# debbiemarkslab/EVcouplings

Measured on AMD Instinct MI355X. Metric: plmc L-BFGS iterations/sec (PLM fit, synthetic MSA), higher is better.
Workload: dtype f32 (forward: f16 hi/lo split couplings on the 2:4 sparse MFMA, f32 accumulation -- in the last iterations of a fit 39-bit fixed-point couplings as five int8 digit planes, exact; backward: 24-bit fixed-point residuals as three int8 digit planes on the int8 MFMA (32-bit / four there), exact int32 acc; 1 GPU; headline: synthetic MSA L=300 q=21 N=50000, theta=0.8, lambda_h=0.01, lambda_J=59.8; parallelism=single GPU

## Files before the change

evcouplings_amd/csrc/plm_host.cpp:

```cpp
#include "../../include/plm_hip.h"
#include "plm_internal.h"
#include "plm_host_util.h"
#include "plm_lbfgs.h"

#include <algorithm>
#include <chrono>
#include <cmath>
#include <cstdarg>
#include <cstdio>
#include <cstdlib>
#include <cstring>
#include <string>
#include <vector>

namespace {

thread_local std::string g_err;

int fail(int code, const char *fmt, ...) {
    char buf[512];
    va_list ap;
    va_start(ap, fmt);
    vsnprintf(buf, sizeof buf, fmt, ap);
    va_end(ap);
// ... 307 lines not shown
    if (d.nblk_own > 0) PLM_HIP(plm_launch_backward(d, c->msa_cm, c->Rt, c->G, nullptr, c->st));
    PLM_HIP(plm_launch_pack_g(d, c->G, c->gsend, c->st));
    PLM_TRY(ctx_collective(c, PLM_COLL_ALLTOALL, c->gsend, c->ghalo, c->g_send.data(), c->g_recv.data()));
    PLM_TRY(group_norms(c));
    PLM_HIP(plm_launch_assemble(d, c->G, d.ksplit, c->ghalo, c->x, c->g, c->prob.lambda_h, c->prob.lambda_j,
                                c->reg_part, 0, 0.f, c->pair_n2, (float)c->prob.lambda_group, c->st));
    PLM_HIP(plm_launch_finish_fx(d, c->fx_part, c->n_fx_part(), nullptr, 0, c->reg_part, plm_reg_parts(d), c->scal,
                                 c->st));
    c->n_evals++;
    return PLM_OK;
}

int ctx_eval_enqueue(plm_ctx *c) {
    const PlmDims &d = c->d;
    if (d.sharded) return ctx_eval_enqueue_sharded(c);
    PLM_HIP(plm_launch_maxabs(d, c->x, c->maxbits, c->jexp, c->st));
    PLM_HIP(plm_launch_expand(d, c->x, nullptr, c->jexp, c->Bt, c->fwd_accurate ? 1 : 0, c->st));
    PLM_TRY(forward_at_x(c));
    PLM_HIP(plm_launch_backward(d, c->msa_cm, c->Rt, c->G, nullptr, c->st));
    const void *Gsrc = c->G;
    int ks_count = d.ksplit, n_shard_nll = 0;
    const double *shard_nll = nullptr;
    if (d.nshards > 1) {
        const size_t slab = plm_slab_bytes(d);
        char *mine = (char *)c->gather + (size_t)d.shard * slab;
        PLM_HIP(plm_launch_slab_reduce(d, c->G, (float *)mine, c->st));
        PLM_HIP(plm_launch_partial_sum(c->fx_part, c->n_fx_part(), (double *)(mine + slab - 256), c->st));
        PLM_HIP(hipStreamSynchronize(c->st));
        if (!c->exchange) return fail(PLM_EINVAL, "n_shards > 1 but no exchange callback set");
        if (c->exchange(c->gather, slab, d.nshards, d.shard, c->exchange_user) != 0)
            return fail(PLM_ECALLBACK, "exchange callback failed");
        Gsrc = c->gather;
        ks_count = 0;
        n_shard_nll = d.nshards;
        shard_nll = (const double *)((char *)c->gather + slab - 256);
    }
    PLM_TRY(group_norms(c));
    PLM_HIP(plm_launch_assemble(d, Gsrc, ks_count, nullptr, c->x, c->g, c->prob.lambda_h, c->prob.lambda_j,
                                c->reg_part, 0, 0.f, c->pair_n2, (float)c->prob.lambda_group, c->st));
    PLM_HIP(plm_launch_finish_fx(d, c->fx_part, c->n_fx_part(), shard_nll, n_shard_nll, c->reg_part,
                                 plm_reg_parts(d), c->scal, c->st));
    c->n_evals++;
    return PLM_OK;
}

bool vp_enabled(const plm_ctx *c) {
    return !(c->prob.flags & PLM_FLAG_JOINT_LBFGS) && (c->d.nshards == 1 || c->d.sharded) && c->prob.lambda_h > 0;
}
int vp_alloc(plm_ctx *c) {
    if (c->hj) return PLM_OK;
    const size_t nsites = (size_t)std::max(std::max(1, (c->d.b16_hi - c->d.b16_lo) * 16),
                                           std::min(c->d.L, c->d.own_hi * 16) - c->d.h_site0);
    PLM_TRY(plm_dalloc((char **)&c->hj, plm_hj_bytes(c->d)));
    PLM_TRY(plm_dalloc((char **)&c->hpart, plm_hpart_bytes(c->d)));
    PLM_TRY(plm_dalloc((char **)&c->gpart, plm_gpart_bytes(c->d)));
    PLM_TRY(plm_dalloc((char **)&c->dpart, plm_gpart_bytes(c->d)));
    PLM_TRY(plm_dalloc(&c->hg2, nsites));
    PLM_TRY(plm_dalloc(&c->hinv, nsites * c->d.Q * c->d.Q));
    PLM_TRY(plm_dalloc(&c->h64, 2 * plm_h64_stride(c->d)));
    PLM_TRY(plm_dalloc(&c->hcnt, plm_h64_stride(c->d)));
    c->hcnt_valid = false;
    PLM_TRY(plm_dalloc((char **)&c->vp_flag, sizeof(PlmVpState)));
    PLM_HIP(hipMemsetAsync(c->vp_flag, 0, sizeof(PlmVpState), c->st));
    for (auto &e : c->vp_ev) PLM_HIP(hipEventCreate(&e));
    for (auto &e : c->gemm_ev) PLM_HIP(hipEventCreate(&e));
    c->vp_hess_age = -1;
    return PLM_OK;
}
int vp_counts(plm_ctx *c) {
    if (!c->hcnt_valid) {
        PLM_HIP(plm_launch_site_counts(c->d, c->msa_cm, c->w, c->hcnt, c->st));
        c->hcnt_valid = true;
    }
    return PLM_OK;
}
int vp_stage1(plm_ctx *c) {
    const PlmDims &d = c->d;
    PLM_TRY(vp_counts(c));
    if (d.sharded) {
        PLM_TRY(ctx_collective(c, PLM_COLL_ALLTOALL, x_rectangles(c), c->xhalo, c->x_send.data(), c->x_recv.data()));
        PLM_HIP(plm_launch_maxabs2(c->x + d.nh_pad_l, d.n_local - d.nh_pad_l, c->xhalo,
                                   d.nx_halo * (int64_t)PLM_BLOCK_FLOATS(d), c->maxbits, c->jexp, d.jexp_bias, c->st));
        PLM_HIP(plm_launch_expand(d, c->x, c->xhalo, c->jexp, c->Bt, c->fwd_accurate ? 1 : 0, c->st));
    } else {
        PLM_HIP(plm_launch_maxabs(d, c->x, c->maxbits, c->jexp, c->st));
        PLM_HIP(plm_launch_expand(d, c->x, nullptr, c->jexp, c->Bt, c->fwd_accurate ? 1 : 0, c->st));
    }
    if (c->gemm_ev[0]) PLM_HIP(hipEventRecord(c->gemm_ev[0], c->st));
    PLM_HIP(plm_launch_forward_store(d, c->msa_rm, c->Bt, c->jexp, c->hj, c->fwd_accurate, c->st));
    PLM_HIP(plm_launch_h64_init(d, c->x, c->h64, c->st));
    return PLM_OK;
}
int vp_counts(plm_ctx *c);
int vp_step_and_residuals(plm_ctx *c, bool refresh) {
    const PlmDims &d = c->d;
    PLM_TRY(vp_counts(c));
    const int full = (refresh || c->vp_hess_age < 0) ? 1 : 0;
    PLM_HIP(plm_launch_hpass(d, c->hj, c->msa_rm, c->w, c->h64, 0, full ? 2 : 1, c->fwd_accurate, nullptr, nullptr, c->hpart,
                             c->gpart, c->dpart, nullptr, PLM_VP_ALWAYS, c->st));
    PLM_HIP(plm_launch_hsolve(d, c->hpart, c->gpart, full, c->x, c->h64, c->prob.lambda_h, 1, c->hinv, c->hg2, c->scal + 5, 0.0,
                              0.0, nullptr, 0, c->hcnt, c->dpart, c->st));
    if (full) c->vp_hess_age = 0;
    PLM_HIP(plm_launch_hpass(d, c->hj, c->msa_rm, c->w, c->h64, 1, 1, c->fwd_accurate, c->Rt, c->fx_part, c->hpart, c->gpart,
                             nullptr, nullptr, PLM_VP_ALWAYS, c->st));
    PLM_HIP(plm_launch_hsolve(d, c->hpart, c->gpart, 0, c->x, c->h64, c->prob.lambda_h, 0, c->hinv, c->hg2, c->scal + 5, 0.0,
                              0.0, nullptr, 0, c->hcnt, c->dpart, c->st));
    return PLM_OK;
// ... 992 lines not shown
        hipError_t e = hipEventRecord(ev[0], c->st);
        if (e == hipSuccess) e = plm_launch_hpass(d, c->hj, c->msa_rm, c->w, c->h64, 0, 2, 0, nullptr, nullptr, c->hpart, c->gpart, c->dpart,
                                                  nullptr, PLM_VP_ALWAYS, c->st);
        if (e == hipSuccess) e = plm_launch_hsolve(d, c->hpart, c->gpart, 1, c->x, c->h64, c->prob.lambda_h, 1, c->hinv, c->hg2, c->scal + 5,
                                                   0.0, 0.0, nullptr, 0, c->hcnt, c->dpart, c->st);
        if (e == hipSuccess) e = hipEventRecord(ev[1], c->st);
        if (e == hipSuccess) e = plm_launch_hpass(d, c->hj, c->msa_rm, c->w, c->h64, 1, 1, 0, c->Rt, c->fx_part, c->hpart, c->gpart, nullptr,
                                                  nullptr, PLM_VP_ALWAYS, c->st);
        if (e == hipSuccess) e = plm_launch_hsolve(d, c->hpart, c->gpart, 0, c->x, c->h64, c->prob.lambda_h, 0, c->hinv, c->hg2, c->scal + 5,
                                                   0.0, 0.0, nullptr, 0, c->hcnt, c->dpart, c->st);
        if (e == hipSuccess) e = hipEventRecord(ev[2], c->st);
        if (e == hipSuccess) e = hipEventSynchronize(ev[2]);
        if (e == hipSuccess && hipEventElapsedTime(&ms, ev[0], ev[1]) == hipSuccess) acc[0] += ms;
        if (e == hipSuccess && hipEventElapsedTime(&ms, ev[1], ev[2]) == hipSuccess) acc[1] += ms;
        if (e != hipSuccess) rc = fail(PLM_EDEVICE, "field position timing: %s", hipGetErrorString(e));
    }
    for (auto &e : ev) (void)hipEventDestroy(e);
    c->vp_hess_age = 0;
    out_ms[0] = (float)(acc[0] / reps);
    out_ms[1] = (float)(acc[1] / reps);
    return rc;
}

static int field_probe_checks(plm_ctx_t *c) {
    if (!c->have_weights) return fail(PLM_EINVAL, "weights not set");
    if (c->d.nshards != 1 || c->d.sharded) return fail(PLM_EUNSUPPORTED, "the field-solver probes run on single-shard contexts");
    if (!vp_enabled(c)) return fail(PLM_EINVAL, "the field-solver probes need a variable-projection context (not joint, lambda_h > 0)");
    return PLM_OK;
}
int plm_ctx_field_position(plm_ctx_t *c, int32_t role, int32_t accurate, int32_t update, int32_t prefill,
                           plm_field_buffers_t *out) {
    if (!c || !out) return fail(PLM_EINVAL, "NULL argument");
    if (role < PLM_FIELD_ROLE_STATS || role > PLM_FIELD_ROLE_RESIDUAL) return fail(PLM_EINVAL, "unknown role %d", (int)role);
    if (!out->gpart || !out->dpart || !out->hpart || !out->hcnt || !out->hinv || !out->g2_site || !out->g2_sum || !out->h64 ||
        !out->nll_part)
        return fail(PLM_EINVAL, "NULL output buffer");
    PLM_TRY(field_probe_checks(c));
    const PlmDims &d = c->d;
    const int64_t nsites = (int64_t)(d.b16_hi - d.b16_lo) * 16, hs = (int64_t)plm_h64_stride(d);
    const int64_t n_g = (int64_t)(plm_gpart_bytes(d) / sizeof(double)), n_h = (int64_t)(plm_hpart_bytes(d) / sizeof(float));
    if (out->n_gpart != n_g || out->n_hpart != n_h || out->n_hcnt != hs || out->n_hinv != nsites * d.Q * d.Q ||
        out->n_g2_site != nsites || out->n_h64 != 2 * hs || out->n_nll_part != c->n_fx_part())
        return fail(PLM_EINVAL, "output buffer sizes do not match the context");
    PLM_HIP(hipSetDevice(c->device));
    PLM_TRY(vp_alloc(c));
    const int full = role == PLM_FIELD_ROLE_HESSIAN ? 1 : 0;
    if (!full && update && c->vp_hess_age < 0) return fail(PLM_EINVAL, "no cached inverse Hessians: run a Hessian position first");
    c->eval_valid = false;
    ctx_set_accurate(c, accurate != 0);
    PLM_TRY(vp_stage1(c));
    if (prefill) {
        PLM_HIP(hipMemsetAsync(c->gpart, 0xFF, plm_gpart_bytes(d), c->st));
        PLM_HIP(hipMemsetAsync(c->dpart, 0xFF, plm_gpart_bytes(d), c->st));
        PLM_HIP(hipMemsetAsync(c->hpart, 0xFF, plm_hpart_bytes(d), c->st));
        PLM_HIP(hipMemsetAsync(c->fx_part, 0xFF, sizeof(double) * c->n_fx_part(), c->st));
        PLM_HIP(hipMemsetAsync(c->h64 + hs, 0xFF, sizeof(double) * hs, c->st));
    }
    if (role == PLM_FIELD_ROLE_RESIDUAL)
        PLM_HIP(plm_launch_hpass(d, c->hj, c->msa_rm, c->w, c->h64, 1, 1, c->fwd_accurate, c->Rt, c->fx_part, c->hpart, c->gpart,
                                 nullptr, nullptr, PLM_VP_ALWAYS, c->st));
    else
        PLM_HIP(plm_launch_hpass(d, c->hj, c->msa_rm, c->w, c->h64, 0, full ? 2 : 1, c->fwd_accurate, nullptr, nullptr, c->hpart,
                                 c->gpart, c->dpart, nullptr, PLM_VP_ALWAYS, c->st));
    PLM_HIP(plm_launch_hsolve(d, c->hpart, c->gpart, full, c->x, c->h64, c->prob.lambda_h, update ? 1 : 0, c->hinv, c->hg2,
                              c->scal + 5, 0.0, 0.0, nullptr, 0, c->hcnt, c->dpart, c->st));
    if (full) c->vp_hess_age = 0;
    PLM_HIP(hipMemcpyAsync(out->gpart, c->gpart, sizeof(double) * n_g, hipMemcpyDeviceToHost, c->st));
    PLM_HIP(hipMemcpyAsync(out->dpart, c->dpart, sizeof(double) * n_g, hipMemcpyDeviceToHost, c->st));
    PLM_HIP(hipMemcpyAsync(out->hpart, c->hpart, sizeof(float) * n_h, hipMemcpyDeviceToHost, c->st));
    PLM_HIP(hipMemcpyAsync(out->hcnt, c->hcnt, sizeof(double) * hs, hipMemcpyDeviceToHost, c->st));
    PLM_HIP(hipMemcpyAsync(out->hinv, c->hinv, sizeof(double) * nsites * d.Q * d.Q, hipMemcpyDeviceToHost, c->st));
    PLM_HIP(hipMemcpyAsync(out->g2_site, c->hg2, sizeof(double) * nsites, hipMemcpyDeviceToHost, c->st));
    PLM_HIP(hipMemcpyAsync(out->g2_sum, c->scal + 5, sizeof(double), hipMemcpyDeviceToHost, c->st));
    PLM_HIP(hipMemcpyAsync(out->h64, c->h64, sizeof(double) * 2 * hs, hipMemcpyDeviceToHost, c->st));
    PLM_HIP(hipMemcpyAsync(out->nll_part, c->fx_part, sizeof(double) * c->n_fx_part(), hipMemcpyDeviceToHost, c->st));
    PLM_HIP(hipStreamSynchronize(c->st));
    return PLM_OK;
}
int plm_ctx_field_solve(plm_ctx_t *c, double tol, int32_t vp_c_prev, int32_t invalidate, int32_t accurate,
                        plm_field_solve_t *res, double *fields, int64_t n_fields) {
    if (!c || !res || !fields) return fail(PLM_EINVAL, "NULL argument");
    if (!(tol >= 0) || vp_c_prev < 0 || vp_c_prev > 11) return fail(PLM_EINVAL, "tol must be >= 0 and vp_c_prev in 0..11");
    PLM_TRY(field_probe_checks(c));
    const PlmDims &d = c->d;
    const int64_t hs = (int64_t)plm_h64_stride(d);
    if (n_fields != hs) return fail(PLM_EINVAL, "fields must hold %lld doubles", (long long)hs);
    static_assert(PLM_FIELD_HIST == PLM_VP_HIST && PLM_FIELD_MAXBLK == PLM_VP_MAXBLK, "plm_field_solve_t mirrors PlmVpState");
    PLM_HIP(hipSetDevice(c->device));
    PLM_TRY(vp_alloc(c));
    c->eval_valid = false;
    ctx_set_accurate(c, accurate != 0);
    c->vp_floor2 = ctx_vp_floor2(c);
    c->vp_c_prev = vp_c_prev;
    if (invalidate) c->vp_hess_age = -1;
    const double tol2 = tol * tol;
    double gh2 = 0;
    PLM_TRY(ctx_eval_vp_run(c, tol2, [&]() -> int { return fetch_scalars(c, 0, 8); }, &gh2));
    PlmVpState S;
    PLM_HIP(hipMemcpyAsync(&S, c->vp_flag, sizeof S, hipMemcpyDeviceToHost, c->st));
    PLM_HIP(hipStreamSynchronize(c->st));
    PLM_HIP(hipMemcpyAsync(fields, c->h64 + (size_t)(S.cur ? hs : 0), sizeof(double) * hs, hipMemcpyDeviceToHost, c->st));
    PLM_HIP(hipStreamSynchronize(c->st));
    memset(res, 0, sizeof *res);
    res->gh2 = gh2;
    res->fx = c->h_scal[0];
    res->nll = c->h_scal[1];
    res->passes = (int32_t)std::lround(c->h_scal[6]);
// ... 659 lines not shown
```

evcouplings_amd/csrc/plm_internal.h:

```cpp
#pragma once
#include <stdint.h>
#include <stddef.h>
#include <hip/hip_runtime.h>

#define PLM_MAX_SHARDS 16
#define PLM_PAD_STATE 127
#define PLM_SEQ_TILE 256
#define PLM_R_EXP 14
#define PLM_BWD_MAXPLANES 4
#define PLM_R_QMAX3 8355000.0f
#define PLM_R_QMAX4 2138000000.0f
#define PLM_BWD_KSTEP 128
#define PLM_BWDW_COLS 9
#define PLM_BWD_ONEHOT_VALUE (-128)

#define PLM_FWD_NG(Q) (((Q) + 2) / 4)
#define PLM_FWD_SPU(Q) (4 * PLM_FWD_NG(Q))
#define PLM_FWD_TILES(Q) (5 * PLM_FWD_NG(Q))

struct PlmDims {
    int N, L, Q;
    int Qc;
    int Np;
    int nb16;
// ... 130 lines not shown
                               hipStream_t st);
hipError_t plm_launch_onehot_rt(const PlmDims &d, const int8_t *msa_rm, const float *w, void *Rt,
                                hipStream_t st);
hipError_t plm_launch_maxabs(const PlmDims &d, const float *x, uint32_t *maxbits, int32_t *jexp,
                             hipStream_t st);
hipError_t plm_launch_expand(const PlmDims &d, const float *x, const float *xhalo, const int32_t *jexp,
                             void *Bt, int exact, hipStream_t st);
hipError_t plm_launch_forward_energy(const PlmDims &d, const int8_t *msa_rm, const void *Bt, const float *x,
                                     const int32_t *jexp, int potentials, int accurate, float *out, hipStream_t st);
hipError_t plm_launch_energy_sum(const PlmDims &d, const float *part, double *out, hipStream_t st);
hipError_t plm_launch_forward_store(const PlmDims &d, const int8_t *msa_rm, const void *Bt, const int32_t *jexp,
                                    float *hj, int exact, hipStream_t st);
int plm_fwd_groups(int q, int exact);
hipError_t plm_launch_hpass(const PlmDims &d, const float *hj, const int8_t *msa_rm, const float *w,
                            const double *h64, int write_rt, int stats, int exact, void *Rt, double *fx_part, float *hpart,
                            double *gpart, double *dpart, const int *state, int cond, hipStream_t st);
#define PLM_VP_HIST 24
#define PLM_VP_MAXBLK 256
struct PlmVpState {
    int done;
    int want_rt;
    int final_skip;
    int passes;
    int cur;
    int pad_;
    double g2_prev;
    double g2_prev2;
    double hist[PLM_VP_HIST];
    int hist_loud[PLM_VP_HIST];
    unsigned char quiet[PLM_VP_MAXBLK];
};
#define PLM_VP_ALWAYS 0
#define PLM_VP_PASS 1
#define PLM_VP_PASS_RT 2
#define PLM_VP_FINAL 3
hipError_t plm_launch_vp_reset(int *state, int want_rt, double *zero3, hipStream_t st);
struct PlmRccl;
int plm_rccl_id(void *id128);
int plm_rccl_version();
int plm_rccl_init(const void *id128, int nranks, int rank, PlmRccl **out);
void plm_rccl_destroy(PlmRccl *p);
int plm_rccl_collective(PlmRccl *p, int op, void *send, void *recv, const int64_t *scounts, const int64_t *rcounts,
                        hipStream_t st);
const char *plm_rccl_error();
hipError_t plm_launch_h64_init(const PlmDims &d, const float *x, double *h64, hipStream_t st);
hipError_t plm_launch_hsolve(const PlmDims &d, const float *hpart, const double *gpart, int full, float *x, double *h64,
                             double lambda_h, int update, double *hinv, double *g2_site, double *g2_out, double tol2,
                             double floor2, int *state, int chain, const double *cnt, const double *dpart, hipStream_t st);
hipError_t plm_launch_site_counts(const PlmDims &d, const int8_t *msa_cm, const float *w, double *cnt, hipStream_t st);
size_t plm_h64_stride(const PlmDims &d);
hipError_t plm_launch_fields_to_x(const PlmDims &d, const double *h64, const int *state, float *x, hipStream_t st);
size_t plm_hj_bytes(const PlmDims &d);
size_t plm_hpart_bytes(const PlmDims &d);
size_t plm_gpart_bytes(const PlmDims &d);
hipError_t plm_launch_backward(const PlmDims &d, const int8_t *msa_cm, const void *Rt, int32_t *G, const int *run,
                               hipStream_t st);
hipError_t plm_launch_slab_reduce(const PlmDims &d, const int32_t *G, float *slab, hipStream_t st);
hipError_t plm_launch_assemble(const PlmDims &d, const void *G, int ks_count, const float *ghalo,
                               const float *x, float *g, float lambda_h, float lambda_j, double *reg_part,
                               int mode, float inv_neff, const float *pair_n2, float lambda_g, hipStream_t st);
hipError_t plm_launch_pair_norms(const PlmDims &d, const float *x, float *n2, hipStream_t st);
#define PLM_BLOCK_FLOATS(d) ((size_t)(d).Q * (d).Q * 256)
hipError_t plm_launch_pack_g(const PlmDims &d, const int32_t *G, float *sendbuf, hipStream_t st);
hipError_t plm_launch_maxabs2(const float *a, int64_t na, const float *b, int64_t nb, uint32_t *maxbits,
                              int32_t *jexp, int jexp_bias, hipStream_t st);
hipError_t plm_launch_finish_fx(const PlmDims &d, const double *fx_part, int n_fx_part,
                                const double *shard_nll, int n_shard_nll, const double *reg_part,
                                int n_reg_part, double *out2 , hipStream_t st);
hipError_t plm_launch_partial_sum(const double *part, int n, double *out, hipStream_t st);
#define PLM_DOT_BLOCKS 1024
hipError_t plm_launch_dots(int npairs, const float *const *a, const float *const *b, int64_t n,
                           double *scratch, double *out, hipStream_t st);
hipError_t plm_launch_lincomb(float *out, float ca, const float *a, float cb, const float *b,
                              int64_t n, hipStream_t st);
hipError_t plm_launch_canon_to_native(const PlmDims &d, const float *xc, float *xn, hipStream_t st);
hipError_t plm_launch_native_to_canon(const PlmDims &d, const float *xn, float *xc, hipStream_t st);
hipError_t plm_launch_fn(const PlmDims &d, const float *jij_canon, float *fn, int a_lo, int g_lo, hipStream_t st);
hipError_t plm_launch_msa_columns(const PlmDims &d, const int8_t *msa_rm, int8_t *msa_cm, int cm_rows, hipStream_t st);
hipError_t plm_launch_compact_gap_blocks(const PlmDims &d, const float *blocks, float *out, hipStream_t st);
hipError_t plm_launch_gap_normalise_pairs(const PlmDims &d, float *fij_canon, double fixed_total, hipStream_t st);
hipError_t plm_launch_align_stats(const int8_t *msa, int n, int L, int gap_state, const int8_t *query, int32_t *seq_gaps,
                                  int32_t *col_gaps, int32_t *ident, hipStream_t st);
size_t plm_bt_bytes(const PlmDims &d);
size_t plm_rt_bytes(const PlmDims &d);
size_t plm_g_bytes(const PlmDims &d);
size_t plm_slab_bytes(const PlmDims &d);
int plm_reg_parts(const PlmDims &d);
bool plm_q_supported(int q);
int plm_q_template(int q);
void plm_pick_tile(int q, int *fm, int *fn);

#define PLM_MAX_BASIS 42
struct PlmVecList {
    const float *v[PLM_MAX_BASIS];
    int n;
};
hipError_t plm_launch_multidot(const PlmVecList &queries, const PlmVecList &basis, int64_t n, double *scratch,
                               double *out, const float *dinv, unsigned wq, unsigned long long wb, hipStream_t st);
struct PlmCoefList {
    float c[PLM_MAX_BASIS];
};
hipError_t plm_launch_multiaxpy(float *out, const PlmVecList &basis, const PlmCoefList &coef, int64_t n,
                                const float *dinv, int first_weighted, hipStream_t st);
hipError_t plm_launch_precond(const PlmDims &d, const float *fv, float neff, float lambda_h, float lambda_j, float *dinv,
                              hipStream_t st);
hipError_t plm_launch_sy_multidot(float *s_new, float *y_new, const float *x, const float *xp, const float *g, const float *gp,
// ... 7 lines not shown
```

evcouplings_amd/csrc/plm_kernels.hip:

```cpp
#include "../../include/plm_hip.h"
#include "plm_internal.h"
#include <math.h>
#include <stdlib.h>
#include <string.h>
#include <mutex>
#include <utility>

typedef _Float16 half8 __attribute__((ext_vector_type(8)));
typedef _Float16 half4 __attribute__((ext_vector_type(4)));
typedef _Float16 half16 __attribute__((ext_vector_type(16)));
typedef float f32x4 __attribute__((ext_vector_type(4)));
typedef int i32x4 __attribute__((ext_vector_type(4)));
typedef unsigned int u32;

#ifndef PLM_DMA_STAGGER_FWD
#define PLM_DMA_STAGGER_FWD 4
#endif
#ifndef PLM_DMA_STAGGER_BWD
#define PLM_DMA_STAGGER_BWD 0
#endif
typedef unsigned long long u64;
#ifndef PLM_ASYNC_A
#define PLM_ASYNC_A 1
#endif
// ... 1123 lines not shown
#define PLM_HSTATS(Q) ((Q) + (Q) * ((Q) + 1) / 2)
__host__ __device__ constexpr int plm_qc_min(int Q) { return Q == 4 ? 2 : Q == 5 ? 5 : Q == 20 ? 6 : Q == 21 ? 21 : 22; }
#ifndef PLM_HESS_SAMPLE
#define PLM_HESS_SAMPLE 32
#endif
#ifndef PLM_NEWTON_CAP
#define PLM_NEWTON_CAP 3.0
#endif
__device__ __forceinline__ float sum_over_g(float v) {
    unsigned u = __float_as_uint(v);
    auto a = __builtin_amdgcn_permlane32_swap(u, u, false, false);
    v = __uint_as_float(a[0]) + __uint_as_float(a[1]);
    u = __float_as_uint(v);
    auto b = __builtin_amdgcn_permlane16_swap(u, u, false, false);
    return __uint_as_float(b[0]) + __uint_as_float(b[1]);
}
__device__ __forceinline__ float log_unbiased(float z) {
    const float l2 = __builtin_amdgcn_logf(z);
    return __builtin_fmaf(l2, -1.904654323148236e-9f, l2 * 0.693147182464599609375f);
}
__device__ __forceinline__ float sel_eq(int x, int a, float if_ne, float if_eq) {
    float out;
    asm("v_cmp_eq_u32 vcc, %1, %2\n\tv_cndmask_b32 %0, %3, %4, vcc" : "=v"(out) : "s"(a), "v"(x), "v"(if_ne), "v"(if_eq) : "vcc");
    return out;
}
__device__ __forceinline__ void sel_eq2(int x, int a, float ne0, float eq0, float ne1, float eq1, float &o0, float &o1) {
    asm("v_cmp_eq_u32 vcc, %2, %3\n\tv_cndmask_b32 %0, %4, %5, vcc\n\tv_cndmask_b32 %1, %6, %7, vcc"
        : "=&v"(o0), "=&v"(o1) : "s"(a), "v"(x), "v"(ne0), "v"(eq0), "v"(ne1), "v"(eq1) : "vcc");
}
__global__ void k_sum_partials(const double *__restrict__ p, int n, double *out);
struct HpassArgs {
    const float4 *hj;
    const int8_t *msa_rm;
    const float *w;
    const double *h;
    int hstride;
    char *Rt;
    double *fx_part;
    float *hpart;
    double *gpart;
    float rscale;
    double *dpart;
    const int *state;
    int cond;
    int sel;
};
__device__ __forceinline__ bool vp_runs(const int *state, int cond) {
    if (!state || cond == PLM_VP_ALWAYS) return true;
    const PlmVpState *S = (const PlmVpState *)state;
    if (cond == PLM_VP_FINAL) return S->final_skip == 0;
    if (S->done) return false;
    return cond == PLM_VP_PASS_RT ? S->want_rt != 0 : S->want_rt == 0;
}
#define PLM_HESS_PARTS(Q) (((Q) == 20 || (Q) == 21) ? 3 : 1)
template <int Q> __host__ __device__ constexpr int hess_entry0(int a) { return a * Q - a * (a - 1) / 2; }
template <int Q> __host__ __device__ constexpr int hess_row_begin(int part) {
    if (part <= 0) return 0;
    if (part >= PLM_HESS_PARTS(Q)) return Q;
    int a = 0;
    while (a < Q && hess_entry0<Q>(a) * PLM_HESS_PARTS(Q) < part * (Q * (Q + 1) / 2)) a++;
    return a;
}
template <int Q> __host__ __device__ constexpr int hess_part_entries() {
    int m = 0;
    for (int p = 0; p < PLM_HESS_PARTS(Q); p++) {
        const int n = hess_entry0<Q>(hess_row_begin<Q>(p + 1)) - hess_entry0<Q>(hess_row_begin<Q>(p));
        m = n > m ? n : m;
    }
    return m;
}
template <int Q, bool WRITE_RT, int STATS, bool XACT>
__global__ __launch_bounds__(512) void k_hpass(PlmDims d, HpassArgs A) {
    extern __shared__ __attribute__((aligned(16))) char smem[];
    constexpr int NH = (STATS == 2) ? Q * (Q + 1) / 2 : 0;
    constexpr int NSP = (STATS == 2) ? PLM_HESS_PARTS(Q) : 1;
    constexpr int NHP = (STATS == 2) ? hess_part_entries<Q>() : 0;
    if (!vp_runs(A.state, A.cond)) return;
    if (A.state) A.h += (size_t)((const PlmVpState *)A.state)->cur * A.hstride;
    const int tid = threadIdx.x, lane = tid & 63;
    const int wave = __builtin_amdgcn_readfirstlane(tid >> 6);
    const int ns1 = (d.nstiles + PLM_HESS_SAMPLE - 1) / PLM_HESS_SAMPLE;
    const int sel = A.sel;
    const int part = (int)blockIdx.x % NSP, bid = (int)blockIdx.x / NSP;
    int row_lo = 0, row_hi = Q;
    if constexpr (NSP > 1) {
        row_lo = part == 0 ? 0 : (part == 1 ? hess_row_begin<Q>(1) : hess_row_begin<Q>(2));
        row_hi = part == 0 ? hess_row_begin<Q>(1) : (part == 1 ? hess_row_begin<Q>(2) : Q);
    }
    const int ent_lo = row_lo * Q - row_lo * (row_lo - 1) / 2, ent_hi = row_hi * Q - row_hi * (row_hi - 1) / 2;
    const int nst = sel == 0 ? d.nstiles : (sel == 1 ? ns1 : d.nstiles - ns1);
    const int kt = bid % nst, b16l = bid / nst;
    if (A.state && A.cond == PLM_VP_PASS && b16l < PLM_VP_MAXBLK && ((const PlmVpState *)A.state)->quiet[b16l]) return;
    const int stile = sel == 0 ? kt : (sel == 1 ? kt * PLM_HESS_SAMPLE : kt + kt / (PLM_HESS_SAMPLE - 1) + 1);
    constexpr int HW = Q > 21 ? 2 : 8;
    constexpr bool sampled = STATS == 2, DIAG = STATS == 3 || (STATS == 2 && Q > 21);
    const int blk = b16l * d.nstiles + stile;
    const int b16 = d.b16_lo + b16l;
    const int r = lane & 15, g = lane >> 4;
    const int s_wave = stile * PLM_SEQ_TILE + wave * 32;
    const int gap = d.gap_mode;
    const int i = b16 * 16 + r;
    const bool site_ok = i < d.L;
    float hv[XACT ? 1 : Q], hl[XACT ? 1 : Q];
    double hd[XACT ? Q : 1];
    auto load_fields = [&](bool opaque) {
        u32 hoff = (u32)(site_ok ? i - d.h_site0 : 0) * Q;
        if (opaque) asm volatile("" : "+v"(hoff));
#pragma unroll
        for (int a = 0; a < Q; a++) {
            const double h64 = site_ok ? A.h[hoff + a] : 0.0;
            if constexpr (XACT) {
                hd[a] = h64;
            } else {
                hv[a] = (float)h64;
                hl[a] = (float)(h64 - (double)hv[a]);
            }
        }
    };
    constexpr bool LDSF = !WRITE_RT && !XACT && (STATS != 2 || Q > 21);
    constexpr size_t STAT_BYTES = (size_t)16 * (8 * Q * sizeof(double) * (DIAG ? 2 : 1) + HW * NHP * sizeof(float));
    float2 *lf = (float2 *)(smem + STAT_BYTES);
    constexpr bool FAST = !WRITE_RT && !XACT && (STATS == 1 || STATS == 3);
    if constexpr (LDSF) {
        for (int k = tid; k < 16 * Q; k += 512) {
            const int ii = b16 * 16 + k / Q;
            const double h64 = ii < d.L ? A.h[(size_t)(ii - d.h_site0) * Q + k % Q] : 0.0;
            const float hi = (float)h64;
            lf[k] = make_float2(hi, (float)(h64 - (double)hi));
        }
        __syncthreads();
    } else if constexpr (!WRITE_RT) load_fields(false);
    float fxl = 0.f;
    double *lg = (double *)smem + ((size_t)wave * 16 + r) * Q;
    double *ld = lg + (size_t)8 * 16 * Q;
    float *lh0 = (float *)((double *)smem + (size_t)8 * 16 * Q * (DIAG ? 2 : 1));
    float *ls = lh0 + ((size_t)wave * 16 + r) * NHP;
    if (STATS) {
        for (int k = lane; k < 16 * Q; k += 64) ((double *)smem)[(size_t)wave * 16 * Q + k] = 0.0;
        if constexpr (sampled)
            if (wave < HW)
                for (int k = lane; k < 16 * NHP; k += 64) lh0[(size_t)wave * 16 * NHP + k] = 0.f;
        if constexpr (DIAG)
            for (int k = lane; k < 16 * Q; k += 64) ((double *)smem)[(size_t)(8 + wave) * 16 * Q + k] = 0.0;
    }
    const char *hj_u = (const char *)(A.hj + ((size_t)blk * 8 + wave) * 2 * Q * 64);
    const u32 lane16 = (u32)lane * 16;
    int m_end = 2;
    asm volatile("" : "+s"(m_end));
#pragma nounroll
    for (int m = 0; m < m_end; m++) {
        if constexpr (WRITE_RT) load_fields(true);
        f32x4 acc[Q];
#pragma unroll
        for (int a = 0; a < Q; a++) {
            const float4 v = *(const float4 *)(hj_u + (size_t)(m * Q + a) * 1024 + lane16);
            acc[a] = (f32x4){v.x, v.y, v.z, v.w};
        }
        float wk[4];
        float izk[4];
        int xk[4];
#pragma unroll
        for (int reg = 0; reg < 4; reg++) {
            const int s = s_wave + 16 * m + 4 * g + reg;
            const int xi = A.msa_rm[(size_t)s * d.Lp32 + i];
            const bool skip = gap && xi == 0;
            const float ws = (skip || !site_ok) ? 0.f : A.w[s];
            float mx = -INFINITY, Z = 0.f, hx = 0.f, zo = 0.f;
            if constexpr (!XACT) {
                u32 foff = (u32)r * Q;
                if constexpr (LDSF) asm volatile("" : "+v"(foff));
#pragma unroll
                for (int a = 0; a < Q; a++) {
                    float fh, fl;
                    if constexpr (LDSF) {
                        const float2 f = lf[foff + a];
                        fh = f.x;
                        fl = f.y;
                    } else {
                        fh = hv[a];
                        fl = hl[a];
                    }
                    const float H = ((gap && a == 0) || (a >= plm_qc_min(Q) && a >= d.Qc)) ? -INFINITY : (acc[a][reg] + fl) + fh;
                    acc[a][reg] = H;
                    mx = fmaxf(mx, H);
                }
                if constexpr (FAST) {
                    const float mxl = -mx * 1.44269502f;
#pragma unroll
                    for (int a = 0; a < Q; a++) {
                        const float ev = __builtin_amdgcn_exp2f(__builtin_fmaf(acc[a][reg], 1.44269502f, mxl));
                        const float evo = sel_eq(xi, a, ev, 0.f);
                        acc[a][reg] = evo;
                        Z += ev;
                        zo += evo;
                    }
                } else {
// ... 10 lines not shown
                }
            } else {
#pragma unroll
                for (int a = 0; a < Q; a++) {
                    const float H = ((gap && a == 0) || a >= d.Qc) ? -INFINITY : acc[a][reg] + (float)hd[a];
                    mx = fmaxf(mx, H);
                }
                const double mxd = (double)mx;
#pragma unroll
                for (int a = 0; a < Q; a++) {
                    const double xs = ((double)acc[a][reg] + hd[a]) - mxd;
                    const double y = xs * 1.4426950408889634;
                    const float yh = (float)y, yl = (float)(y - (double)yh);
                    const float rr = __builtin_amdgcn_exp2f(yh);
                    const float ev = ((gap && a == 0) || a >= d.Qc) ? 0.f : __builtin_fmaf(rr, yl * 0.693147182464599609375f, rr);
                    float evo;
                    sel_eq2(xi, a, hx, (float)xs, ev, 0.f, hx, evo);
                    acc[a][reg] = ev;
                    Z += ev;
                    zo += evo;
                }
            }
            const float invZ = 1.f / Z;
            if (WRITE_RT && ws > 0.f) fxl -= ws * (hx - log_unbiased(Z));
            const float mpo = -(zo * invZ);
            if constexpr (FAST) {
                if (ws != 0.f) {
                    unsafeAtomicAdd(&lg[xi], (double)(ws * mpo));
                    if constexpr (STATS == 3) {
                        const float px = 1.f + mpo;
                        unsafeAtomicAdd(&ld[xi], (double)(ws * px * px));
                    }
                }
                wk[reg] = ws * invZ;
                izk[reg] = invZ;
                xk[reg] = xi;
            } else {
#pragma unroll
            for (int a = 0; a < Q; a++) acc[a][reg] = sel_eq(xi, a, acc[a][reg] * invZ, mpo);
            wk[reg] = ws;
            xk[reg] = xi;
            }
            asm volatile("" : "+v"(xk[reg]));
            if constexpr (XACT) __builtin_amdgcn_sched_barrier(0);
        }
        if constexpr (STATS != 0) {
            int idx = 0;
#pragma unroll
            for (int a = 0; a < Q; a++) {
                float t[4], ga = 0.f;
#pragma unroll
                for (int k = 0; k < 4; k++) {
                    t[k] = wk[k] * acc[a][k];
                    ga += t[k];
                }
#ifndef PLM_EXP_NOGRAD
                if (NSP == 1 || part == 0) unsafeAtomicAdd(&lg[a], (double)ga);
#else
                fxl += ga;
#endif
                if constexpr (DIAG) {
                    float da = 0.f;
                    if constexpr (FAST) {
#pragma unroll
                        for (int k = 0; k < 4; k++) da = fmaf(t[k] * acc[a][k], izk[k], da);
                    } else {
#pragma unroll
                    for (int k = 0; k < 4; k++) {
                        const bool obs = xk[k] == a;
                        da = fmaf(t[k] + (obs ? wk[k] : 0.f), acc[a][k] + (obs ? 1.f : 0.f), da);
                    }
                    }
#ifndef PLM_EXP_NOGRAD
                    unsafeAtomicAdd(&ld[a], (double)da);
#else
                    fxl += da;
#endif
                }
#ifndef PLM_EXP_NOHESS
                if (STATS == 2 && wave < HW && a >= row_lo && a < row_hi) {
                    idx = a * Q - a * (a - 1) / 2 - ent_lo;
#pragma unroll
                    for (int k = 0; k < 4; k++) t[k] += (xk[k] == a) ? wk[k] : 0.f;
#pragma unroll
                    for (int b = a; b < Q; b++) {
                        float v = 0.f;
#pragma unroll
                        for (int k = 0; k < 4; k++) v = fmaf(t[k], acc[b][k] + ((xk[k] == b) ? 1.f : 0.f), v);
#ifndef PLM_EXP_NOSWAP
                        v = sum_over_g(v);
#endif
#ifndef PLM_EXP_NOLDS
                        if (g == 0) __builtin_amdgcn_ds_faddf(LDS_FPTR(&ls[idx]), v, 0, 0, false);
#else
                        fxl += v;
#endif
                        ++idx;
                    }
                }
#endif
            }
        }
        if constexpr (WRITE_RT) {
            __builtin_amdgcn_sched_barrier(0);
            const int s64 = stile * 4 + (wave >> 1);
            const int Gq = 2 * (wave & 1) + m;
            char *rt_u = A.Rt + rt_slot(d, 0, s64, b16l * Q, 0);
            const size_t rt_plane = (size_t)d.nst128 * d.nnfl * 2048;
            const u32 slot16 = (u32)(Gq * 16 + r) * 16;
#pragma unroll
            for (int reg = 0; reg < 4; reg++) {
                wk[reg] *= A.rscale;
                asm volatile("" : "+v"(xk[reg]));
            }
            const bool four = d.nplanes == 4;
            auto planes_of_state = [&](int a, u32 (&pl)[PLM_BWD_MAXPLANES]) {
                u32 x[4];
#pragma unroll
                for (int reg = 0; reg < 4; reg++)
                    x[reg] = digits_of(wk[reg] * acc[a][reg], four);
                planes_of4(x[0], x[1], x[2], x[3], pl);
            };
#pragma unroll
            for (int q4 = 0; q4 + 4 <= Q; q4 += 4) {
                u32 pl[4][PLM_BWD_MAXPLANES];
#pragma unroll
                for (int k = 0; k < 4; k++) planes_of_state(q4 + k, pl[k]);
                const u32 off = (u32)(q4 + g) * 2048 + slot16;
#pragma unroll
                for (int p = 0; p < PLM_BWD_MAXPLANES; p++) {
                    if (p >= d.nplanes) break;
                    auto s02 = __builtin_amdgcn_permlane32_swap(pl[0][p], pl[2][p], false, false);
                    auto s13 = __builtin_amdgcn_permlane32_swap(pl[1][p], pl[3][p], false, false);
                    auto t0 = __builtin_amdgcn_permlane16_swap(s02[0], s13[0], false, false);
                    auto t1 = __builtin_amdgcn_permlane16_swap(s02[1], s13[1], false, false);
                    *(uint4 *)(rt_u + p * rt_plane + off) = make_uint4(t0[0], t0[1], t1[0], t1[1]);
                }
                __builtin_amdgcn_sched_barrier(0);
            }
#pragma unroll
            for (int a = Q - Q % 4; a < Q; a++) {
                u32 pl[PLM_BWD_MAXPLANES];
                planes_of_state(a, pl);
#pragma unroll
                for (int p = 0; p < PLM_BWD_MAXPLANES; p++)
                    if (p < d.nplanes) *(u32 *)(rt_u + p * rt_plane + (u32)a * 2048 + slot16 + 4 * g) = pl[p];
            }
        }
    }
    __syncthreads();
    if constexpr (STATS != 0) {
        if (NSP == 1 || part == 0) {
            double *gout = A.gpart + (size_t)blk * 16 * Q;
            for (int k = tid; k < 16 * Q; k += 512) {
                double v = 0;
#pragma unroll
                for (int wv = 0; wv < 8; wv++) v += ((const double *)smem)[(size_t)wv * 16 * Q + k];
                gout[k] = v;
            }
        }
        if constexpr (DIAG) {
            double *dout = A.dpart + (size_t)blk * 16 * Q;
            for (int k = tid; k < 16 * Q; k += 512) {
                double v = 0;
#pragma unroll
                for (int wv = 0; wv < 8; wv++) v += ((const double *)smem)[(size_t)(8 + wv) * 16 * Q + k];
                dout[k] = v;
            }
        }
        if constexpr (sampled) {
            float *out = A.hpart + (size_t)blk * 16 * NH;
            const int ne = ent_hi - ent_lo;
            for (int k = tid; k < 16 * ne; k += 512) {
                const int site = k / ne, e = k - site * ne;
                float v = 0.f;
#pragma unroll
                for (int wv = 0; wv < HW; wv++) v += lh0[((size_t)wv * 16 + site) * NHP + e];
                out[site * NH + ent_lo + e] = v;
            }
        }
    }
    if constexpr (WRITE_RT) {
        __syncthreads();
        const double tot = block_reduce_sum((double)fxl, (double *)smem);
        if (tid == 0) A.fx_part[blk] = tot;
    }
}
hipError_t plm_launch_hpass(const PlmDims &d, const float *hj, const int8_t *msa_rm, const float *w,
                            const double *h64, int write_rt, int stats, int exact, void *Rt, double *fx_part, float *hpart,
                            double *gpart, double *dpart, const int *state, int cond, hipStream_t st) {
    if (d.b16_hi <= d.b16_lo) return hipSuccess;
    const int nb = d.b16_hi - d.b16_lo, ns1 = (d.nstiles + PLM_HESS_SAMPLE - 1) / PLM_HESS_SAMPLE;
    const dim3 block(512);
    HpassArgs A{(const float4 *)hj, msa_rm, w, h64, (int)plm_h64_stride(d), (char *)Rt, fx_part,
                hpart, gpart, d.rscale, dpart, state, cond, 0};
#define HP_LAUNCH(QQ, WW, SS)                                                                          \
    {                                                                                                  \
        const dim3 grid((A.sel == 0 ? d.nstiles : (A.sel == 1 ? ns1 * ((SS) == 2 ? PLM_HESS_PARTS(QQ) : 1) : d.nstiles - ns1)) * nb); \
        const size_t lds = (size_t)16 * (8 * (QQ) * sizeof(double) * (((SS) == 3 || ((SS) == 2 && (QQ) > 21)) ? 2 : 1) + \
                                         ((SS) == 2 ? ((QQ) > 21 ? 2 : 8) * hess_part_entries<QQ>() : 0) * sizeof(float)) + \
                           (size_t)16 * (QQ) * sizeof(float2);           \
        {                                                                                              \
            hipError_t e = exact ? plm_allow_lds<k_hpass<QQ, WW, SS, true>>(lds) : plm_allow_lds<k_hpass<QQ, WW, SS, false>>(lds); \
            if (e != hipSuccess) return e;                                                             \
        }                                                                                              \
        if (exact) hipLaunchKernelGGL((k_hpass<QQ, WW, SS, true>), grid, block, lds, st, d, A);        \
        else hipLaunchKernelGGL((k_hpass<QQ, WW, SS, false>), grid, block, lds, st, d, A);             \
    }
#define HP_CASE(QQ)                                                                                    \
    case QQ:                                                                                           \
        if (write_rt && stats == 2) return hipErrorInvalidValue;    \
        else if (write_rt && stats == 0) HP_LAUNCH(QQ, true, 0)                                        \
        else if (write_rt) HP_LAUNCH(QQ, true, 1)                                                      \
        else if (stats == 2) {                                                                         \
            if (!dpart) return hipErrorInvalidValue;                                                   \
                         \
            A.sel = 1;                                                                                 \
            HP_LAUNCH(QQ, false, 2)                                                                    \
            A.sel = 2;                                                                                 \
            if (d.nstiles > ns1) HP_LAUNCH(QQ, false, 3)                                               \
        } else HP_LAUNCH(QQ, false, 1)                                                                 \
        break;
    switch (d.Q) {
        HP_CASE(32)
        HP_CASE(21)
        HP_CASE(20)
        HP_CASE(5)
        HP_CASE(4)
    default:
        return hipErrorInvalidValue;
    }
#undef HP_CASE
#undef HP_LAUNCH
    return hipGetLastError();
}
size_t plm_hpart_bytes(const PlmDims &d) {
    return (size_t)d.nstiles * (d.b16_hi - d.b16_lo) * 16 * (d.Q * (d.Q + 1) / 2) * sizeof(float);
}
size_t plm_h64_stride(const PlmDims &d) {
    const size_t nsites = (size_t)std::max(std::max(1, (d.b16_hi - d.b16_lo) * 16), std::min(d.L, d.own_hi * 16) - d.h_site0);
    return nsites * d.Q;
}
size_t plm_gpart_bytes(const PlmDims &d) { return (size_t)d.nstiles * (d.b16_hi - d.b16_lo) * 16 * d.Q * sizeof(double); }

template <int Q>
__global__ __launch_bounds__(256) void k_site_counts(PlmDims d, const int8_t *__restrict__ msa_cm, const float *__restrict__ w,
                                                    double *__restrict__ cnt) {
    __shared__ double red[4];
    const int il = blockIdx.x, i = d.h_site0 + il;
    double acc[Q];
#pragma unroll
    for (int a = 0; a < Q; a++) acc[a] = 0.0;
    if (i < d.L)
        for (int s = threadIdx.x; s < d.N; s += 256) {
            const int x = msa_cm[(size_t)i * d.Np + s];
            const double ws = (d.gap_mode && x == 0) ? 0.0 : (double)w[s];
#pragma unroll
            for (int a = 0; a < Q; a++) acc[a] += (x == a) ? ws : 0.0;
        }
#pragma unroll
    for (int a = 0; a < Q; a++) {
        const double t = block_reduce_sum(acc[a], red);
        if (threadIdx.x == 0) cnt[(size_t)il * Q + a] = t;
        __syncthreads();
    }
}
hipError_t plm_launch_site_counts(const PlmDims &d, const int8_t *msa_cm, const float *w, double *cnt, hipStream_t st) {
    const int nsites = (d.b16_hi - d.b16_lo) * 16;
    if (nsites <= 0) return hipSuccess;
    switch (d.Q) {
    case 32: hipLaunchKernelGGL(k_site_counts<32>, dim3(nsites), dim3(256), 0, st, d, msa_cm, w, cnt); break;
    case 21: hipLaunchKernelGGL(k_site_counts<21>, dim3(nsites), dim3(256), 0, st, d, msa_cm, w, cnt); break;
    case 20: hipLaunchKernelGGL(k_site_counts<20>, dim3(nsites), dim3(256), 0, st, d, msa_cm, w, cnt); break;
    case 5: hipLaunchKernelGGL(k_site_counts<5>, dim3(nsites), dim3(256), 0, st, d, msa_cm, w, cnt); break;
    case 4: hipLaunchKernelGGL(k_site_counts<4>, dim3(nsites), dim3(256), 0, st, d, msa_cm, w, cnt); break;
    default: return hipErrorInvalidValue;
    }
    return hipGetLastError();
}

template <int Q>
__global__ __launch_bounds__(64) void k_hsolve(PlmDims d, const float *__restrict__ hpart,
                                              const double *__restrict__ gpart, int full,
                                              float *__restrict__ x, double *__restrict__ h64,
                                              double lambda_h, int update,
                                              double *__restrict__ hinv, double *__restrict__ g2_site,
                                              double tol_site2, const int *__restrict__ state, int chain, int hstride,
                                              const double *__restrict__ cnt, const double *__restrict__ dpart) {
    constexpr int NVF = PLM_HSTATS(Q);
    const PlmVpState *S = (const PlmVpState *)state;
// ... 1535 lines not shown
```

Baseline: 111.7 iterations/s.

## Split Hessian pass across wave-group blocks with per-wave partials and tile-sum kernel

For Q=20/21, the Hessian-stats pass no longer splits rows across three blocks. It splits the 8 waves of a tile across WP smaller blocks (default 8 blocks of one wave). Each wave writes its gradient and Hessian partials to an extra scratch region appended to hpart, and a new k_hess_tile_sums kernel adds the 8 per-wave slices into the per-tile buffers. This is meant to raise occupancy and parallelism and avoid the redundant row-split work, at the cost of a larger hpart allocation, extra global traffic and one more kernel launch.

Result: no change. 112.7 iterations/s, median of 6 (+0.9%).

```diff
diff --git a/evcouplings_amd/csrc/plm_host.cpp b/evcouplings_amd/csrc/plm_host.cpp
--- a/evcouplings_amd/csrc/plm_host.cpp
+++ b/evcouplings_amd/csrc/plm_host.cpp
@@ -383,7 +383,7 @@
     const size_t nsites = (size_t)std::max(std::max(1, (c->d.b16_hi - c->d.b16_lo) * 16),
                                            std::min(c->d.L, c->d.own_hi * 16) - c->d.h_site0);
     PLM_TRY(plm_dalloc((char **)&c->hj, plm_hj_bytes(c->d)));
-    PLM_TRY(plm_dalloc((char **)&c->hpart, plm_hpart_bytes(c->d)));
+    PLM_TRY(plm_dalloc((char **)&c->hpart, plm_hpart_alloc_bytes(c->d)));
     PLM_TRY(plm_dalloc((char **)&c->gpart, plm_gpart_bytes(c->d)));
     PLM_TRY(plm_dalloc((char **)&c->dpart, plm_gpart_bytes(c->d)));
     PLM_TRY(plm_dalloc(&c->hg2, nsites));
@@ -1482,7 +1482,7 @@
     if (prefill) {
         PLM_HIP(hipMemsetAsync(c->gpart, 0xFF, plm_gpart_bytes(d), c->st));
         PLM_HIP(hipMemsetAsync(c->dpart, 0xFF, plm_gpart_bytes(d), c->st));
-        PLM_HIP(hipMemsetAsync(c->hpart, 0xFF, plm_hpart_bytes(d), c->st));
+        PLM_HIP(hipMemsetAsync(c->hpart, 0xFF, plm_hpart_alloc_bytes(d), c->st));
         PLM_HIP(hipMemsetAsync(c->fx_part, 0xFF, sizeof(double) * c->n_fx_part(), c->st));
         PLM_HIP(hipMemsetAsync(c->h64 + hs, 0xFF, sizeof(double) * hs, c->st));
     }
diff --git a/evcouplings_amd/csrc/plm_internal.h b/evcouplings_amd/csrc/plm_internal.h
--- a/evcouplings_amd/csrc/plm_internal.h
+++ b/evcouplings_amd/csrc/plm_internal.h
@@ -206,6 +206,7 @@
 hipError_t plm_launch_fields_to_x(const PlmDims &d, const double *h64, const int *state, float *x, hipStream_t st);
 size_t plm_hj_bytes(const PlmDims &d);
 size_t plm_hpart_bytes(const PlmDims &d);
+size_t plm_hpart_alloc_bytes(const PlmDims &d);
 size_t plm_gpart_bytes(const PlmDims &d);
 hipError_t plm_launch_backward(const PlmDims &d, const int8_t *msa_cm, const void *Rt, int32_t *G, const int *run,
                                hipStream_t st);
diff --git a/evcouplings_amd/csrc/plm_kernels.hip b/evcouplings_amd/csrc/plm_kernels.hip
--- a/evcouplings_amd/csrc/plm_kernels.hip
+++ b/evcouplings_amd/csrc/plm_kernels.hip
@@ -1199,7 +1199,19 @@
     if (S->done) return false;
     return cond == PLM_VP_PASS_RT ? S->want_rt != 0 : S->want_rt == 0;
 }
-#define PLM_HESS_PARTS(Q) (((Q) == 20 || (Q) == 21) ? 3 : 1)
+#ifndef PLM_HESS_WPARTS
+#define PLM_HESS_WPARTS 8
+#endif
+static_assert(PLM_HESS_WPARTS == 0 || PLM_HESS_WPARTS == 2 || PLM_HESS_WPARTS == 4 || PLM_HESS_WPARTS == 8, "wave parts: 0 (row split), 2, 4 or 8");
+#define PLM_HESS_WP(Q) (((Q) == 20 || (Q) == 21) ? PLM_HESS_WPARTS : 0)
+#define PLM_HESS_PARTS(Q) ((((Q) == 20 || (Q) == 21) && PLM_HESS_WPARTS == 0) ? 3 : 1)
+__host__ __device__ inline size_t hess_wave_h_offset(const PlmDims &d) {
+    return (size_t)d.nstiles * (d.b16_hi - d.b16_lo) * 16 * (d.Q * (d.Q + 1) / 2) * sizeof(float);
+}
+__host__ __device__ inline size_t hess_wave_g_offset(const PlmDims &d) {
+    const size_t ns1 = (d.nstiles + PLM_HESS_SAMPLE - 1) / PLM_HESS_SAMPLE;
+    return hess_wave_h_offset(d) + ns1 * (d.b16_hi - d.b16_lo) * 8 * 16 * (d.Q * (d.Q + 1) / 2) * sizeof(float);
+}
 template <int Q> __host__ __device__ constexpr int hess_entry0(int a) { return a * Q - a * (a - 1) / 2; }
 template <int Q> __host__ __device__ constexpr int hess_row_begin(int part) {
     if (part <= 0) return 0;
@@ -1217,20 +1229,23 @@
     return m;
 }
 template <int Q, bool WRITE_RT, int STATS, bool XACT>
-__global__ __launch_bounds__(512) void k_hpass(PlmDims d, HpassArgs A) {
+__global__ __launch_bounds__((STATS == 2 && PLM_HESS_WP(Q)) ? 512 / PLM_HESS_WP(Q) : 512) void k_hpass(PlmDims d, HpassArgs A) {
     extern __shared__ __attribute__((aligned(16))) char smem[];
     constexpr int NH = (STATS == 2) ? Q * (Q + 1) / 2 : 0;
-    constexpr int NSP = (STATS == 2) ? PLM_HESS_PARTS(Q) : 1;
+    constexpr int WP = (STATS == 2) ? PLM_HESS_WP(Q) : 0;
+    constexpr int NWV = WP ? 8 / WP : 8;
+    constexpr int NSP = (STATS == 2) ? (WP ? WP : PLM_HESS_PARTS(Q)) : 1;
     constexpr int NHP = (STATS == 2) ? hess_part_entries<Q>() : 0;
     if (!vp_runs(A.state, A.cond)) return;
     if (A.state) A.h += (size_t)((const PlmVpState *)A.state)->cur * A.hstride;
     const int tid = threadIdx.x, lane = tid & 63;
-    const int wave = __builtin_amdgcn_readfirstlane(tid >> 6);
+    const int lwave = __builtin_amdgcn_readfirstlane(tid >> 6);
     const int ns1 = (d.nstiles + PLM_HESS_SAMPLE - 1) / PLM_HESS_SAMPLE;
     const int sel = A.sel;
     const int part = (int)blockIdx.x % NSP, bid = (int)blockIdx.x / NSP;
+    const int wave = WP ? part * NWV + lwave : lwave;
     int row_lo = 0, row_hi = Q;
-    if constexpr (NSP > 1) {
+    if constexpr (NSP > 1 && WP == 0) {
         row_lo = part == 0 ? 0 : (part == 1 ? hess_row_begin<Q>(1) : hess_row_begin<Q>(2));
         row_hi = part == 0 ? hess_row_begin<Q>(1) : (part == 1 ? hess_row_begin<Q>(2) : Q);
     }
@@ -1265,7 +1280,7 @@
         }
     };
     constexpr bool LDSF = !WRITE_RT && !XACT && (STATS != 2 || Q > 21);
-    constexpr size_t STAT_BYTES = (size_t)16 * (8 * Q * sizeof(double) * (DIAG ? 2 : 1) + HW * NHP * sizeof(float));
+    constexpr size_t STAT_BYTES = (size_t)16 * (NWV * Q * sizeof(double) * (DIAG ? 2 : 1) + (WP ? NWV : HW) * NHP * sizeof(float));
     float2 *lf = (float2 *)(smem + STAT_BYTES);
     constexpr bool FAST = !WRITE_RT && !XACT && (STATS == 1 || STATS == 3);
     if constexpr (LDSF) {
@@ -1278,17 +1293,17 @@
         __syncthreads();
     } else if constexpr (!WRITE_RT) load_fields(false);
     float fxl = 0.f;
-    double *lg = (double *)smem + ((size_t)wave * 16 + r) * Q;
-    double *ld = lg + (size_t)8 * 16 * Q;
-    float *lh0 = (float *)((double *)smem + (size_t)8 * 16 * Q * (DIAG ? 2 : 1));
-    float *ls = lh0 + ((size_t)wave * 16 + r) * NHP;
+    double *lg = (double *)smem + ((size_t)lwave * 16 + r) * Q;
+    double *ld = lg + (size_t)NWV * 16 * Q;
+    float *lh0 = (float *)((double *)smem + (size_t)NWV * 16 * Q * (DIAG ? 2 : 1));
+    float *ls = lh0 + ((size_t)lwave * 16 + r) * NHP;
     if (STATS) {
-        for (int k = lane; k < 16 * Q; k += 64) ((double *)smem)[(size_t)wave * 16 * Q + k] = 0.0;
+        for (int k = lane; k < 16 * Q; k += 64) ((double *)smem)[(size_t)lwave * 16 * Q + k] = 0.0;
         if constexpr (sampled)
             if (wave < HW)
-                for (int k = lane; k < 16 * NHP; k += 64) lh0[(size_t)wave * 16 * NHP + k] = 0.f;
+                for (int k = lane; k < 16 * NHP; k += 64) lh0[(size_t)lwave * 16 * NHP + k] = 0.f;
         if constexpr (DIAG)
-            for (int k = lane; k < 16 * Q; k += 64) ((double *)smem)[(size_t)(8 + wave) * 16 * Q + k] = 0.0;
+            for (int k = lane; k < 16 * Q; k += 64) ((double *)smem)[(size_t)(NWV + lwave) * 16 * Q + k] = 0.0;
     }
     const char *hj_u = (const char *)(A.hj + ((size_t)blk * 8 + wave) * 2 * Q * 64);
     const u32 lane16 = (u32)lane * 16;
@@ -1405,10 +1420,11 @@
 #pragma unroll
                 for (int k = 0; k < 4; k++) {
                     t[k] = wk[k] * acc[a][k];
+                    if constexpr (WP != 0) asm("" : "+v"(t[k]));
                     ga += t[k];
                 }
 #ifndef PLM_EXP_NOGRAD
-                if (NSP == 1 || part == 0) unsafeAtomicAdd(&lg[a], (double)ga);
+                if (WP || NSP == 1 || part == 0) unsafeAtomicAdd(&lg[a], (double)ga);
 #else
                 fxl += ga;
 #endif
@@ -1502,7 +1518,13 @@
         }
     }
     __syncthreads();
-    if constexpr (STATS != 0) {
+    if constexpr (WP != 0) {
+        const size_t wslot = ((size_t)b16l * ns1 + kt) * 8 + wave;
+        double *gout = (double *)((char *)A.hpart + hess_wave_g_offset(d)) + wslot * 16 * Q;
+        for (int k = lane; k < 16 * Q; k += 64) gout[k] = ((const double *)smem)[(size_t)lwave * 16 * Q + k];
+        float *out = (float *)((char *)A.hpart + hess_wave_h_offset(d)) + wslot * 16 * NH;
+        for (int k = lane; k < 16 * NH; k += 64) out[k] = lh0[(size_t)lwave * 16 * NHP + k];
+    } else if constexpr (STATS != 0) {
         if (NSP == 1 || part == 0) {
             double *gout = A.gpart + (size_t)blk * 16 * Q;
             for (int k = tid; k < 16 * Q; k += 512) {
@@ -1539,19 +1561,52 @@
         if (tid == 0) A.fx_part[blk] = tot;
     }
 }
+#define PLM_HESS_TSPLIT 4
+template <int Q>
+__global__ __launch_bounds__(256) void k_hess_tile_sums(PlmDims d, float *__restrict__ hpart, double *__restrict__ gpart,
+                                                       const int *__restrict__ state, int cond) {
+    constexpr int NH = Q * (Q + 1) / 2;
+    if (!vp_runs(state, cond)) return;
+    const int ns1 = (d.nstiles + PLM_HESS_SAMPLE - 1) / PLM_HESS_SAMPLE;
+    const int sub = (int)blockIdx.x % PLM_HESS_TSPLIT, bid = (int)blockIdx.x / PLM_HESS_TSPLIT;
+    const int kt = bid % ns1, b16l = bid / ns1;
+    if (state && cond == PLM_VP_PASS && b16l < PLM_VP_MAXBLK && ((const PlmVpState *)state)->quiet[b16l]) return;
+    const size_t blk = (size_t)b16l * d.nstiles + (size_t)kt * PLM_HESS_SAMPLE, wslot = ((size_t)b16l * ns1 + kt) * 8;
+    const double *gw = (const double *)((const char *)hpart + hess_wave_g_offset(d)) + wslot * 16 * Q;
+    const float *hw = (const float *)((const char *)hpart + hess_wave_h_offset(d)) + wslot * 16 * NH;
+    const int k0 = sub * 256 + (int)threadIdx.x;
+    for (int k = k0; k < 16 * NH; k += 256 * PLM_HESS_TSPLIT) {
+        float u[8], v = 0.f;
+#pragma unroll
+        for (int wv = 0; wv < 8; wv++) u[wv] = hw[(size_t)wv * 16 * NH + k];
+#pragma unroll
+        for (int wv = 0; wv < 8; wv++) v += u[wv];
+        hpart[blk * 16 * NH + k] = v;
+    }
+    for (int k = k0; k < 16 * Q; k += 256 * PLM_HESS_TSPLIT) {
+        double u[8], v = 0;
+#pragma unroll
+        for (int wv = 0; wv < 8; wv++) u[wv] = gw[(size_t)wv * 16 * Q + k];
+#pragma unroll
+        for (int wv = 0; wv < 8; wv++) v += u[wv];
+        gpart[blk * 16 * Q + k] = v;
+    }
+}
 hipError_t plm_launch_hpass(const PlmDims &d, const float *hj, const int8_t *msa_rm, const float *w,
                             const double *h64, int write_rt, int stats, int exact, void *Rt, double *fx_part, float *hpart,
                             double *gpart, double *dpart, const int *state, int cond, hipStream_t st) {
     if (d.b16_hi <= d.b16_lo) return hipSuccess;
     const int nb = d.b16_hi - d.b16_lo, ns1 = (d.nstiles + PLM_HESS_SAMPLE - 1) / PLM_HESS_SAMPLE;
-    const dim3 block(512);
     HpassArgs A{(const float4 *)hj, msa_rm, w, h64, (int)plm_h64_stride(d), (char *)Rt, fx_part,
                 hpart, gpart, d.rscale, dpart, state, cond, 0};
 #define HP_LAUNCH(QQ, WW, SS)                                                                          \
     {                                                                                                  \
-        const dim3 grid((A.sel == 0 ? d.nstiles : (A.sel == 1 ? ns1 * ((SS) == 2 ? PLM_HESS_PARTS(QQ) : 1) : d.nstiles - ns1)) * nb); \
-        const size_t lds = (size_t)16 * (8 * (QQ) * sizeof(double) * (((SS) == 3 || ((SS) == 2 && (QQ) > 21)) ? 2 : 1) + \
-                                         ((SS) == 2 ? ((QQ) > 21 ? 2 : 8) * hess_part_entries<QQ>() : 0) * sizeof(float)) + \
+         \
+        constexpr int wp = (SS) == 2 ? PLM_HESS_WP(QQ) : 0, nwv = wp ? 8 / wp : 8;                      \
+        const dim3 block(64 * nwv);                                                                    \
+        const dim3 grid((A.sel == 0 ? d.nstiles : (A.sel == 1 ? ns1 * ((SS) == 2 ? (wp ? wp : PLM_HESS_PARTS(QQ)) : 1) : d.nstiles - ns1)) * nb); \
+        const size_t lds = (size_t)16 * (nwv * (QQ) * sizeof(double) * (((SS) == 3 || ((SS) == 2 && (QQ) > 21)) ? 2 : 1) + \
+                                         ((SS) == 2 ? ((QQ) > 21 ? 2 : nwv) * hess_part_entries<QQ>() : 0) * sizeof(float)) + \
                            (size_t)16 * (QQ) * sizeof(float2);           \
         {                                                                                              \
             hipError_t e = exact ? plm_allow_lds<k_hpass<QQ, WW, SS, true>>(lds) : plm_allow_lds<k_hpass<QQ, WW, SS, false>>(lds); \
@@ -1570,7 +1625,9 @@
                          \
             A.sel = 1;                                                                                 \
             HP_LAUNCH(QQ, false, 2)                                                                    \
-            A.sel = 2;                                                                                 \
+            if constexpr (PLM_HESS_WP(QQ) != 0)                                                        \
+                hipLaunchKernelGGL(k_hess_tile_sums<QQ>, dim3(ns1 * nb * PLM_HESS_TSPLIT), dim3(256), 0, st, d, hpart, gpart, state, cond); \
+            A.sel = 2;                                                                              \
             if (d.nstiles > ns1) HP_LAUNCH(QQ, false, 3)                                               \
         } else HP_LAUNCH(QQ, false, 1)                                                                 \
         break;
@@ -1589,6 +1646,11 @@
 }
 size_t plm_hpart_bytes(const PlmDims &d) {
     return (size_t)d.nstiles * (d.b16_hi - d.b16_lo) * 16 * (d.Q * (d.Q + 1) / 2) * sizeof(float);
+}
+size_t plm_hpart_alloc_bytes(const PlmDims &d) {
+    if (!PLM_HESS_WPARTS || (d.Q != 20 && d.Q != 21)) return plm_hpart_bytes(d);
+    const size_t ns1 = (d.nstiles + PLM_HESS_SAMPLE - 1) / PLM_HESS_SAMPLE;
+    return hess_wave_g_offset(d) + ns1 * (d.b16_hi - d.b16_lo) * 8 * 16 * d.Q * sizeof(double);
 }
 size_t plm_h64_stride(const PlmDims &d) {
     const size_t nsites = (size_t)std::max(std::max(1, (d.b16_hi - d.b16_lo) * 16), std::min(d.L, d.own_hi * 16) - d.h_site0);
```
